# mingfeisun/DeepMimic_mujoco

Measured on AMD Instinct MI355X. Metric: env-steps/sec, higher is better.
Workload: dtype f64

## Files before the change

deepmimic_mujoco_amd/csrc/slot_kernel.h:

```cpp
#pragma once

#include <cstddef>

#include "env_kernel.h"

namespace dm {

constexpr int SLOTS = 4, SW = 16;
#ifndef DM_SLOT_MAXROWS
#define DM_SLOT_MAXROWS 40
#endif
constexpr int SLOT_MAXROWS = DM_SLOT_MAXROWS, SLOT_MAXLIMROWS = 16, SLOT_MAXCON = 13, SLOT_MAXFRAME = 8, SLOT_MAXCAND = 32, SLOT_BOXSLOTS = 3;
constexpr int SLOT_EXTROWS = SLOT_MAXROWS - 2 * SW;
static_assert(SLOT_EXTROWS == 8 || SLOT_EXTROWS == 0, "the partial third row set holds eight rows (or is absent)");
constexpr int PAIR_PASSES = MAXPAIR / SW;
static_assert(MAXPAIR <= 128 && NG <= 16, "a candidate word holds the pair number in 7 bits and both geom numbers in 4 bits each");
constexpr int DOF_PASSES = (NV + SW - 1) / SW, HINGE_PASSES = (NU + SW - 1) / SW, Q_PASSES = (NQ + SW - 1) / SW, ENT_PASSES = (310 + SW - 1) / SW;

#ifndef DM_SLOT_ASSUME
#define DM_SLOT_ASSUME 31
#endif
#ifndef DM_SLOT_A10T
#define DM_SLOT_A10T 1
#endif
// ... 594 lines not shown
        int tot_rows, tot_con;
        const int r0 = nrow + row_exclusive_scan(pc.n * rows_per, sl, lane, &tot_rows);
        const int c0 = ncon + row_exclusive_scan(pc.n, sl, lane, &tot_con);
        const unsigned fmask = dmw::row_ballot(pc.n > 0, lane);
        const int fi = nfr + __builtin_popcount(fmask & below);
        nfr += __builtin_popcount(fmask);
        if (pc.n > 0) {
          R fr[9];
          make_frame(fr, pc.nrm, pc.hint);
          if (fi < SLOT_MAXFRAME) { R* o = W.frm[fi]; for (int t = 0; t < 6; t++) o[t] = fr[t]; }
          for (int k = 0; k < pc.n; k++) {
            const int ci = c0 + k, rk = r0 + k * rows_per;
            if (ci >= SLOT_MAXCON || fi >= SLOT_MAXFRAME || rk + rows_per > MAXR) { ovf |= (ci >= SLOT_MAXCON || fi >= SLOT_MAXFRAME) ? 4 : 8; continue; }
            R cdist, cpos[3];
            if (pc.boxslot >= 0) { const R* o = W.boxc[pc.boxslot][k]; cdist = o[0]; cpos[0] = o[1]; cpos[1] = o[2]; cpos[2] = o[3]; }
            else if (k == 0) { cdist = pc.d0; cpos[0] = pc.p0[0]; cpos[1] = pc.p0[1]; cpos[2] = pc.p0[2]; }
            else { cdist = pc.d1; cpos[0] = pc.p1[0]; cpos[1] = pc.p1[1]; cpos[2] = pc.p1[2]; }
            R* o = W.con[ci];
            o[0] = cpos[0]; o[1] = cpos[1]; o[2] = cpos[2]; o[3] = cdist;
            W.coni[ci] = pidx | (fi << 8);
            for (int q = 0; q < rows_per; q++) W.rowi[rk + q] = ROW_CONTACT | (ci << 8) | (q << 16) | (dim << 20);
          }
        }
        nrow += tot_rows; ncon += tot_con;
      }
    }
  }
  if (nrow > MAXR) ovf |= 8;
  if (dmw::row_ballot(ovf != 0, lane) != 0u) { ovf |= 64; nrow = 0; ncon = 0; }
  if (sl == 0) { s.nefc = nrow; s.ncon = ncon; }
  dmw::sync();
  SLOT_RSTAMP(21)
#undef SLOT_RSTAMP
  return nrow;
}

template <int I, int NVEC, class R>
struct SlotSolveLTStep {
  static DM_DEV void run(R (*x)[NV], const R* qLD, const R* cur) {
    R nxt[14];
    dmw::reload_fence();
    load_factor_row<I - 1>(nxt, qLD);
    dmw::sched_fence();
#pragma unroll
    for (int v = 0; v < NVEC; v++) {
#pragma unroll
      for (int a = 1; a < 14; a++) { const int j = TOPO.dof_anc[I][a]; if (j >= 0) x[v][j] -= cur[a] * x[v][I]; }
      dmw::pin_value(x[v][TOPO.dof_anc[I][1]]);
    }
    SlotSolveLTStep<I - 1, NVEC, R>::run(x, qLD, nxt);
  }
};
template <int NVEC, class R> struct SlotSolveLTStep<0, NVEC, R> { static DM_DEV void run(R (*)[NV], const R*, const R*) {} };
template <int NVEC, class R> DM_DEV void slot_solve_LT(R (*x)[NV], const R* qLD) {
  R cur[14];
  dmw::reload_fence();
  load_factor_row<NV - 1>(cur, qLD);
  SlotSolveLTStep<NV - 1, NVEC, R>::run(x, qLD, cur);
}

template <int D, class R>
DM_DEV void slot_load_dof_operands(R* dst, const SlotShared<R>& s) {
  if constexpr (D < NV) {
#pragma unroll
    for (int r = 0; r < 6; r++) dst[r] = s.cdof[D][r];
    dst[6] = s.qvel[D]; dst[7] = s.qws[D];
  }
}
template <int D, int NS, class R>
struct SlotRowStep {
  static DM_DEV void run(R (*y)[NV], RowAcc<R>* ra, const SlotShared<R>& s, const R* cur) {
    R nxt[8];
    dmw::reload_fence();
    slot_load_dof_operands<D + 1>(nxt, s);
    dmw::sched_fence();
#pragma unroll
    for (int k = 0; k < NS; k++) {
      const int pb = (int)(D < 32 ? (ra[k].plus_lo >> D) & 1u : (ra[k].plus_hi >> (D - 32)) & 1u);
      const int mb = (int)(D < 32 ? (ra[k].minus_lo >> D) & 1u : (ra[k].minus_hi >> (D - 32)) & 1u);
      R j = ra[k].w[0] * cur[0] + ra[k].w[1] * cur[1] + ra[k].w[2] * cur[2] + ra[k].w[3] * cur[3] + ra[k].w[4] * cur[4] + ra[k].w[5] * cur[5];
      j = (j + ra[k].w7) * (R)(pb - mb);
      ra[k].vel += j * cur[6]; ra[k].jws += j * cur[7];
      y[k][D] = j;
      dmw::pin_value(ra[k].vel); dmw::pin_value(ra[k].jws);
    }
    SlotRowStep<D + 1, NS, R>::run(y, ra, s, nxt);
  }
};
template <int NS, class R> struct SlotRowStep<NV, NS, R> { static DM_DEV void run(R (*)[NV], RowAcc<R>*, const SlotShared<R>&, const R*) {} };

template <int CC, int NS, class R, bool T10 = false>
DM_DEV void slot_acol(R (*AR)[16 * NS], const R (*y)[NV]) {
#pragma unroll
  for (int k = 0; k < (T10 && CC < 16 ? 1 : NS); k++) {
    R acc0 = 0, acc1 = 0;
#pragma unroll
    for (int d = 0; d + 8 <= NV; d += 8) dmw::row_fmac8<CC % 16>(acc0, acc1, &y[CC / 16][d], &y[k][d]);
#pragma unroll
    for (int d = NV / 8 * 8; d < NV; d += 2) { dmw::row_fmac_old<CC % 16>(acc0, y[CC / 16][d], y[k][d]); dmw::row_fmac_old<CC % 16>(acc1, y[CC / 16][d + 1], y[k][d + 1]); }
    AR[k][CC] = acc0 + acc1;
  }
}
template <int C, int NS, class R, bool T10 = false>
struct SlotACols {
  static DM_DEV void run(R (*AR)[16 * NS], const R (*y)[NV], int nmax) {
    if constexpr (C < 16 * NS) {
      slot_acol<C, NS, R, T10>(AR, y); slot_acol<C + 1, NS, R, T10>(AR, y); slot_acol<C + 2, NS, R, T10>(AR, y); slot_acol<C + 3, NS, R, T10>(AR, y);
      if (C + 4 < nmax) SlotACols<C + 4, NS, R, T10>::run(AR, y, nmax);
    }
  }
};
// ... 186 lines not shown
  for (int r6 = 0; r6 < 6; r6++) ra.w[r6] = w[r6];
  ra.w7 = w7; ra.w8 = 0; ra.vel = 0; ra.jws = 0;
  ra.plus_lo = (unsigned)mplus; ra.plus_hi = (unsigned)(mplus >> 32); ra.minus_lo = (unsigned)mminus; ra.minus_hi = (unsigned)(mminus >> 32);
}

template <class R, int NS, bool PROF = false>
DM_DEV void slot_constraint(const DevModel<R>& M, SlotShared<R>& s, int sl_in, int lane_in, int nefc, int nmax, int& ovf, const DebugOut* dbg, long long* prof = 0) {
  const int sl = DM_SLOT_LANE_AT(4, sl_in), lane = dmw::launder(lane_in);
  long long pt0 = 0, pt1 = 0, pt_enter = 0;
  if (PROF) { pt0 = dmw::clk(); pt_enter = pt0; }
#define SLOT_STAMP(k) if constexpr (NS == 1) { DM_MARK("slot_constraint_ns1_" #k); } else if constexpr (NS == 2) { DM_MARK("slot_constraint_ns2_" #k); } else { DM_MARK("slot_constraint_ns3_" #k); } if (PROF) { pt1 = dmw::clk(); prof[k] += pt1 - pt0; pt0 = pt1; }
  constexpr bool EXT = NS == 3;
  constexpr int NF = EXT ? 2 : NS;
  constexpr int NC = 16 * NF;
  constexpr int NX = EXT ? SLOT_EXTROWS : 1;
  if constexpr (NS == 1) { DM_MARK("slot_constraint_ns1_rows"); } else if constexpr (NS == 2) { DM_MARK("slot_constraint_ns2_rows"); } else { DM_MARK("slot_constraint_ns3_rows"); }
  R y[NF + 1][NV];
  RowAcc<R> ra[NF];
  bool active[NF];
  R pos[NF], margin[NF], dA[NF], rscale[NF];
#pragma unroll
  for (int k = 0; k < NF; k++) {
    const int r = sl + 16 * k;
    active[k] = r < nefc;
    slot_row_setup(M, s, r, active[k], ra[k], pos[k], margin[k], dA[k], rscale[k]);
  }
  {
    R cur[8];
    dmw::reload_fence();
    slot_load_dof_operands<0>(cur, s);
    SlotRowStep<0, NF, R>::run(y, ra, s, cur);
  }
#pragma unroll
  for (int d = 0; d < NV; d++) y[NF][d] = s.tau[d];
  if (dbg) {
#pragma unroll
    for (int k = 0; k < NF; k++) if (active[k]) {
      double* o = dbg->out + (34 * 34 + 34 * 3 + 42 + 3) + (sl + 16 * k) * (34 + 6);
#pragma unroll
      for (int d = 0; d < NV; d++) o[d] = (double)y[k][d];
    }
  }
  SLOT_STAMP(8)
  R Rr[NF], aref[NF], f[NF];
#pragma unroll
  for (int k = 0; k < NF; k++) {
    const R imp = impedance(M, pos[k] - margin[k]);
    Rr[k] = fmax(R(DM_MINVAL), (1 - imp) * dA[k] / imp);
    if (rscale[k] != R(1)) Rr[k] = fmax(R(DM_MINVAL), rscale[k] * Rr[k]);
    aref[k] = -M.B * ra[k].vel - M.K * imp * (pos[k] - margin[k]);
    const R jar = ra[k].jws - aref[k];
    f[k] = (active[k] && jar < 0) ? -jar / Rr[k] : R(0);
  }
  slot_solve_LT<NF + 1>(y, s.r2.qLD);
#pragma unroll
  for (int d = 0; d < NV; d++) {
    const R sc = s.dsq[d];
#pragma unroll
    for (int k = 0; k <= NF; k++) { y[k][d] *= sc; dmw::pin_value(y[k][d]); }
  }
  if (dbg) {
    R x[NV];
#pragma unroll
    for (int d = 0; d < NV; d++) x[d] = y[NF][d] * s.dsq[d];
    solve_L(x, s.r2.qLD);
    if (sl == 0) {
#pragma unroll
      for (int d = 0; d < NV; d++) dbg->out[34 * 34 + 34 + d] = (double)x[d];
    }
  }
  R bb[NF];
#pragma unroll
  for (int k = 0; k < NF; k++) {
    R acc0 = 0, acc1 = 0;
#pragma unroll
    for (int d = 0; d < NV; d++) { if (d & 1) acc1 += y[k][d] * y[NF][d]; else acc0 += y[k][d] * y[NF][d]; }
    bb[k] = active[k] ? (acc0 + acc1) - aref[k] : R(0);
  }
  R y3[EXT ? NV : 1];
  bool active3 = false;
  R Rr3 = 0, f3 = 0, bb3 = 0;
  if constexpr (EXT) {
    dmw::sync();
    if (sl == 0) {
#pragma unroll
      for (int d = 0; d < NV; d++) s.tau[d] = y[NF][d];
    }
    const int r3 = 2 * SW + (sl >> 1);
    active3 = (sl & 1) == 0 && r3 < nefc;
    RowAcc<R> ra3[1];
    R pos3, margin3, dA3, rscale3;
    slot_row_setup(M, s, r3, active3, ra3[0], pos3, margin3, dA3, rscale3);
    R yy[1][NV];
    {
      R cur[8];
      dmw::reload_fence();
      slot_load_dof_operands<0>(cur, s);
      SlotRowStep<0, 1, R>::run(yy, ra3, s, cur);
    }
    const R imp = impedance(M, pos3 - margin3);
    Rr3 = fmax(R(DM_MINVAL), (1 - imp) * dA3 / imp);
    if (rscale3 != R(1)) Rr3 = fmax(R(DM_MINVAL), rscale3 * Rr3);
    const R aref3 = -M.B * ra3[0].vel - M.K * imp * (pos3 - margin3);
    const R jar = ra3[0].jws - aref3;
    f3 = (active3 && jar < 0) ? -jar / Rr3 : R(0);
    slot_solve_LT<1>(yy, s.r2.qLD);
    dmw::sync();
    R acc0 = 0, acc1 = 0;
#pragma unroll
    for (int d = 0; d < NV; d++) {
      y3[d] = yy[0][d] * s.dsq[d]; dmw::pin_value(y3[d]);
      if (d & 1) acc1 += y3[d] * s.tau[d]; else acc0 += y3[d] * s.tau[d];
    }
    bb3 = active3 ? (acc0 + acc1) - aref3 : R(0);
  }
  R U[EXT ? 2 : 1][NX], B3[NX];
  R diag3 = 1;
  if constexpr (EXT) {
#pragma unroll
    for (int j = 0; j < NX; j++) { U[0][j] = 0; U[1][j] = 0; B3[j] = 0; dmw::pin_value(U[0][j]); dmw::pin_value(U[1][j]); dmw::pin_value(B3[j]); }
    dmw::dpp_settle();
    SlotExtCols<0, R>::run(U, B3, y, y3, nmax - 2 * SW);
    R dg = 1;
#pragma unroll
    for (int j = 0; j < NX; j++) { if (sl == 2 * j) { B3[j] += active3 ? Rr3 : R(0); dg = B3[j]; } }
    diag3 = active3 ? dg : R(1);
    R* y3lds = &s.qd.o.qacc[0];
    if ((sl & 1) == 0) {
#pragma unroll
      for (int d = 0; d < NV; d++) y3lds[d * SLOT_EXTROWS + (sl >> 1)] = y3[d];
    }
  }
  SLOT_STAMP(9)
  R AR[NF][NC];
#pragma unroll
  for (int k = 0; k < NF; k++)
#pragma unroll
    for (int c = 0; c < NC; c++) { AR[k][c] = 0; dmw::pin_value(AR[k][c]); }
  dmw::dpp_settle();
  constexpr bool T10 = NS == 2 && DM_SLOT_A10T;
  SlotACols<0, NF, R, T10>::run(AR, y, nmax);
  if constexpr (T10) slot_a10_transpose(AR, s, sl);
  R diag[NF];
#pragma unroll
  for (int k = 0; k < NF; k++) {
    R dg = 1;
#pragma unroll
    for (int c = 0; c < 16; c++) { if (sl == c) { AR[k][16 * k + c] += active[k] ? Rr[k] : R(0); dg = AR[k][16 * k + c]; } }
    diag[k] = active[k] ? dg : R(1);
  }
  SLOT_STAMP(10)
  typedef decltype(dmw::park(R(0))) ParkedR;
  ParkedR ypark[NF == 2 ? NF : 1][NF == 2 ? NV : 1];
  if constexpr (NF == 2) {
    if constexpr (!EXT) {
      if (sl == 0) {
#pragma unroll
        for (int d = 0; d < NV; d++) s.tau[d] = y[NF][d];
      }
// ... 106 lines not shown
      if constexpr (EXT) nf3 = conv ? nfprev3 : nf3;
      const bool go = (int)act & (int)!conv;
      iter += go ? 1 : 0;
      anybad = (int)anybad | ((int)go & (int)bad2);
      frozen = (int)frozen | (int)conv;
      chg = chg2;
      more = dmw::ballot(!frozen) != 0ull;
      if (PROF) prof[6] += 1;
    }
  }
#pragma unroll
  for (int k = 0; k < NF; k++) f[k] = -nf[k];
  f3 = -nf3;
  if (PROF && NS >= 2) { prof[22] += dmw::clk() - pt0; }
  if (PROF && NS == 3) { prof[27] += dmw::clk() - pt0; }
  SLOT_STAMP(12)
  if (PROF) { prof[14] += nmax; prof[15] += 1; }
  if (dmw::row_ballot(anybad, lane) != 0u) ovf |= 16 | 64;
  if (dbg) {
#pragma unroll
    for (int k = 0; k < NF; k++) if (active[k]) {
      double* o = dbg->out + (34 * 34 + 34 * 3 + 42 + 3) + (sl + 16 * k) * (34 + 6) + 34;
      o[0] = (double)pos[k]; o[1] = (double)margin[k]; o[2] = (double)Rr[k]; o[3] = (double)aref[k]; o[4] = (double)bb[k]; o[5] = (double)f[k];
    }
  }
  R fy3[EXT ? NV : 1];
  if constexpr (EXT) {
    const R* y3lds = &s.qd.o.qacc[0];
    const R f3a = active3 ? f3 : R(0);
#pragma unroll
    for (int d = 0; d < NV; d++) { fy3[d] = ((sl & 1) == 0 ? y3lds[d * SLOT_EXTROWS + (sl >> 1)] : R(0)) * f3a; dmw::pin_value(fy3[d]); }
  }
  if constexpr (NF == 2) {
    dmw::sync();
#pragma unroll
    for (int d = 0; d < NV; d++) y[NF][d] = s.tau[d];
  }
#pragma unroll
  for (int k = 0; k < NF; k++) {
    const R fk = active[k] ? f[k] : R(0);
#pragma unroll
    for (int d = 0; d < NV; d++) { if constexpr (NF == 2) y[k][d] = dmw::unpark(ypark[k][d]); y[k][d] *= fk; dmw::pin_value(y[k][d]); }
  }
  R ws[NV];
#pragma unroll
  for (int d = 0; d < NV; d++) { ws[d] = 0; dmw::pin_value(ws[d]); }
  R one = 1;
  dmw::pin_value(one);
  dmw::dpp_settle();
  SlotAssemble<0, NF, R>::run(ws, y, one, nmax);
  if constexpr (EXT) SlotExtAssemble<0, R>::run(ws, fy3, one, nmax - 2 * SW);
#pragma unroll
  for (int d = 0; d < NV; d++) ws[d] = (ws[d] + y[NF][d]) * s.dsq[d];
  solve_L(ws, s.r2.qLD);
  if (sl == 0) {
#pragma unroll
    for (int d = 0; d < NV; d++) s.qd.o.qacc[d] = ws[d];
    s.solver_iter = iter;
  }
  dmw::sync();
  SLOT_STAMP(13)
  if (PROF && NS >= 2) prof[24] += dmw::clk() - pt_enter;
  if (PROF && NS == 3) prof[26] += dmw::clk() - pt_enter;
#undef SLOT_STAMP
}

#if !defined(DM_WAVE_TESTBENCH)
template <class R, int MAXR>
static __device__ __noinline__ int slot_rows_call(const DevModel<R>* M, SlotShared<R>* s, int sl, int lane, int* ovf) {
  int o = *ovf;
  const int n = slot_rows<R, false, MAXR>(*dmw::in_constant(M), *dmw::in_lds(s), sl, lane, o, (long long*)0);
  *ovf = o;
  return n;
}
#endif

template <class R>
DM_DEV void slot_smooth_solve(SlotShared<R>& s, int sl, const DebugOut* dbg) {
  R x[1][NV];
#pragma unroll
  for (int d = 0; d < NV; d++) x[0][d] = s.tau[d];
  slot_solve_LT<1>(x, s.r2.qLD);
#pragma unroll
  for (int d = 0; d < NV; d++) { x[0][d] *= s.dsq[d]; dmw::pin_value(x[0][d]); }
#pragma unroll
  for (int d = 0; d < NV; d++) x[0][d] = (R(0) + x[0][d]) * s.dsq[d];
  solve_L(x[0], s.r2.qLD);
  if (sl == 0) {
#pragma unroll
    for (int d = 0; d < NV; d++) { s.qd.o.qacc[d] = x[0][d]; if (dbg) dbg->out[34 * 34 + 34 + d] = (double)x[0][d]; }
    s.solver_iter = 0;
  }
  dmw::sync();
}

template <class R, bool PROF = false, bool CARRY = false, int MAXR = 2 * SW>
DM_DEV void slot_forward(const DevModel<R>& M, SlotShared<R>& s, const SlotTables& tb, int sl, int lane, const LaneTopo& lt, R* xip, int& ovf, const DebugOut* dbg, long long* prof = 0) {
  long long t0 = 0, t1 = 0;
  if (PROF) t0 = dmw::clk();
#define SLOT_FSTAMP(k) if (PROF) { t1 = dmw::clk(); prof[k] += t1 - t0; t0 = t1; }
  DM_MARK("slot_kinematics");
  bool skip_kin = false;
  if constexpr (CARRY) {
    skip_kin = dmw::ballot(s.kin_ok() != R(0)) == ~0ull;
    dmw::sync();
    if (sl == 0) s.kin_ok() = R(0);
  }
  if (!skip_kin) slot_kinematics(M, s, sl, lt, xip);
  SLOT_FSTAMP(0)
  if (dbg) { for (int e = sl; e < NV * NV; e += SW) dbg->out[e] = 0; dmw::sync(); }
  DM_MARK("slot_bias");
  slot_bias(M, s, tb, sl, lt);
  SLOT_FSTAMP(1)
  if (dbg) {
    for (int c = 0; c < DOF_PASSES; c++) { const int d = sl + SW * c; if (d < NV) dbg->out[34 * 34 + d] = (double)(-M.dof_damping[d] * s.qvel[d] + s.act[d] - s.tau[d]); }
  }
  DM_MARK("slot_mass_factor");
  slot_mass_matrix<R, PROF>(M, s, tb, sl, lt, dbg, prof);
  SLOT_FSTAMP(2)
  DM_MARK("slot_rows");
  int nefc = 0;
#if !defined(DM_WAVE_TESTBENCH)
  if (!PROF && (M.enable_contact || M.enable_limit)) nefc = slot_rows_call<R, MAXR>(&M, &s, sl, lane, &ovf);
  else
#endif
  if (M.enable_contact || M.enable_limit) nefc = slot_rows<R, PROF, MAXR>(M, s, sl, lane, ovf, prof);
  else { if (sl == 0) { s.nefc = 0; s.ncon = 0; } dmw::sync(); }
  SLOT_FSTAMP(3)
  DM_MARK("slot_constraint");
  const int nmax = rows_max(nefc);
  if (nmax == 0) slot_smooth_solve(s, sl, dbg);
#ifdef DM_FORCE_EXT
  else if (nmax > 0 && MAXR > 2 * SW) slot_constraint<R, MAXR > 2 * SW ? 3 : 2, PROF>(M, s, sl, lane, nefc, nmax > 2 * SW ? nmax : 2 * SW + 1, ovf, dbg, prof);
#endif
  else if (nmax <= 16) slot_constraint<R, 1, PROF>(M, s, sl, lane, nefc, nmax, ovf, dbg, prof);
  else if (nmax <= 2 * SW) { slot_constraint<R, 2, PROF>(M, s, sl, lane, nefc, nmax, ovf, dbg, prof); if (PROF) prof[7] += 1; }
  else if constexpr (MAXR > 2 * SW) { slot_constraint<R, 3, PROF>(M, s, sl, lane, nefc, nmax, ovf, dbg, prof); if (PROF) { prof[7] += 1; prof[25] += 1; } }
  SLOT_FSTAMP(4)
  DM_MARK("slot_forward_end");
#undef SLOT_FSTAMP
// ... 9 lines not shown
```

deepmimic_mujoco_amd/csrc/slot_step.h:

```cpp
#pragma once

#include "env_step.h"
#include "slot_kernel.h"

namespace dm {

template <class R> struct DofVec { R r[DOF_PASSES]; };

template <class R>
DM_DEV void slot_integrate_pos(SlotShared<R>& s, const DofVec<R>& x0q, int sl, R h) {
  const R q0 = dmw::row_bcast<3>(x0q.r[0]), q1 = dmw::row_bcast<4>(x0q.r[0]), q2 = dmw::row_bcast<5>(x0q.r[0]), q3 = dmw::row_bcast<6>(x0q.r[0]);
  if (sl < 3) s.qpos[sl] = x0q.r[0] + h * s.tau[sl];
  else if (sl == 3) {
    R ax[3] = {s.tau[3], s.tau[4], s.tau[5]}, q[4] = {q0, q1, q2, q3}, qr[4];
    const R angle = h * normalize3(ax);
    if (angle == R(0)) { qr[0] = 1; qr[1] = qr[2] = qr[3] = 0; } else axisangle2quat(qr, ax, angle);
    normalize4(q);
    quat_mul(q, q, qr);
    s.qpos[3] = q[0]; s.qpos[4] = q[1]; s.qpos[5] = q[2]; s.qpos[6] = q[3];
  } else if (sl >= 7) s.qpos[sl] = x0q.r[0] + h * s.tau[sl - 1];
#pragma unroll
  for (int c = 1; c < Q_PASSES; c++) { const int i = sl + SW * c; if (i < NQ) s.qpos[i] = x0q.r[c] + h * s.tau[i - 1]; }
}

// ... 55 lines not shown
    if (i < NQ) s.qpos[i] = B.qpos[(size_t)env * NQ + i];
    if (i < NV) { s.qvel[i] = B.qvel[(size_t)env * NV + i]; s.qws[i] = B.qws[(size_t)env * NV + i]; s.act[i] = 0; }
  }
  if (sl == 0) { s.status = 0; s.nefc = 0; s.ncon = 0; s.solver_iter = 0; }
  dmw::sync();
  if (action) {
#pragma unroll
    for (int c = 0; c < HINGE_PASSES; c++) {
      const int u = sl + SW * c;
      if (u < NU) {
        const R a = ctrl_of_action(M, B, env, u, (R)action[(size_t)env * NU + u], s.qpos[7 + u], s.qvel[6 + u], n_substeps);
        if (live) B.ctrl[(size_t)env * NU + u] = a;
        s.act[u + 6] = act_force(M, u + 6, a);
      }
    }
  }
  dmw::sync_mem();
}

template <class R, bool CARRY = false>
DM_DEV void slot_spd_control(const DevModel<R>& M, const Batch<R>& B, SlotShared<R>& s, const SlotTables& tb, int env, int sl, const LaneTopo& lt, bool live,
                             const DofVec<R>& qbar, const DofVec<R>& vbar) {
  const R h = M.timestep;
#pragma unroll
  for (int c = 0; c < DOF_PASSES; c++) { const int d = sl + SW * c; if (d < NV) s.act[d] = 0; }
  dmw::sync();
  R xip[3];
  bool skip_kin = false;
  if constexpr (CARRY) {
    skip_kin = dmw::ballot(s.kin_ok() != R(0)) == ~0ull;
    dmw::sync();
    if (sl == 0) s.kin_ok() = R(0);
  }
  if (!skip_kin) slot_kinematics(M, s, sl, lt, xip);
  slot_bias(M, s, tb, sl, lt);
  slot_mass_matrix<R, false, true>(M, s, tb, sl, lt, (const DebugOut*)0);
  R pd[DOF_PASSES], kd[DOF_PASSES];
#pragma unroll
  for (int c = 0; c < DOF_PASSES; c++) {
    const int d = sl + SW * c;
    pd[c] = 0; kd[c] = 0;
    if (d >= 6 && d < NV) {
      const R q = s.qpos[d + 1], v = s.qvel[d];
      kd[c] = M.kd[d];
      pd[c] = M.kp[d] * (qbar.r[c] - q - h * v) + kd[c] * (vbar.r[c] - v);
      s.tau[d] += pd[c];
    }
  }
  dmw::sync();
  {
    R x[1][NV];
#pragma unroll
    for (int d = 0; d < NV; d++) x[0][d] = s.tau[d];
    slot_solve_LT<1>(x, s.r2.qLD);
#pragma unroll
    for (int d = 0; d < NV; d++) { x[0][d] *= s.qd.o.dinv[d]; dmw::pin_value(x[0][d]); }
    solve_L(x[0], s.r2.qLD);
    if (sl == 0) {
#pragma unroll
      for (int d = 0; d < NV; d++) s.qd.o.qacc[d] = x[0][d];
    }
  }
  dmw::sync();
#pragma unroll
  for (int c = 0; c < DOF_PASSES; c++) {
    const int d = sl + SW * c;
    if (d >= 6 && d < NV) {
      const R ct = spd_ctrl(M, d, pd[c], kd[c], s.qd.o.qacc[d], h);
      if (live) B.ctrl[(size_t)env * NU + (d - 6)] = ct;
      s.act[d] = act_force(M, d, ct);
    }
  }
  dmw::sync_mem();
}

template <class R>
DM_DEV void slot_store_state(const Batch<R>& B, SlotShared<R>& s, int env, int sl, bool live) {
  if (!live) return;
#pragma unroll
  for (int c = 0; c < Q_PASSES; c++) {
    const int i = sl + SW * c;
    if (i < NQ) B.qpos[(size_t)env * NQ + i] = s.qpos[i];
    if (i < NV) { B.qvel[(size_t)env * NV + i] = s.qvel[i]; B.qws[(size_t)env * NV + i] = s.qws[i]; }
  }
}

template <class R>
DM_DEV void slot_reset_env(const DevModel<R>& M, const Batch<R>& B, SlotShared<R>& s, int env, int sl, bool doit, int mode, int hard) {
  const int ep = B.episode[env];
  const int genv = B.env_offset + env;
  const int idx = reset_draw(B, env, ep);
  if (doit) {
#pragma unroll
    for (int c = 0; c < Q_PASSES; c++) {
      const int i = sl + SW * c;
      if (i < NQ) {
        R q, v = 0;
        reset_element(M, B, mode, idx, genv, ep, i, q, v);
        s.qpos[i] = q;
        if (i < NV) s.qvel[i] = v;
      }
      if (hard && i < NV) s.qws[i] = 0;
    }
  }
  dmw::sync_mem();
  if (doit && sl == 0) reset_commit(B, env, ep, mode, hard, idx);
}
template <class R>
DM_DEV void slot_reset_env_clips(const DevModel<R>& M, const Batch<R>& B, const ClipArgs<R>& C, SlotShared<R>& s, int env, int sl, bool doit, int mode, int hard) {
  const int c = C.episode_clip(B, env, B.episode[env], mode, hard);
// ... 320 lines not shown
```

deepmimic_mujoco_amd/csrc/wave.h:

```cpp
#pragma once

#if defined(DM_WAVE_TESTBENCH)
#include "wave_testbench.h"
#else
#include <hip/hip_runtime.h>

#define DM_DEV __device__ __forceinline__
#define DM_DEV_NOINLINE __device__ __noinline__
#ifndef DM_NO_STATIC_CALLS
#define DM_STATIC_CALLS 1
#define DM_DEV_CALL64 static __device__ __noinline__
#else
#define DM_DEV_CALL64 __device__ __noinline__
#endif
#define DM_CONSTANT __device__ constexpr

namespace dmw {
DM_DEV int lane() { return (int)(threadIdx.x & 63u); }
DM_DEV void sync() { __builtin_amdgcn_fence(__ATOMIC_SEQ_CST, "wavefront"); __builtin_amdgcn_wave_barrier(); }
DM_DEV void sync_mem() { __syncthreads(); }
DM_DEV unsigned long long ballot(bool p) { return __ballot(p); }
DM_DEV int shfl_i(int v, int src) { return __shfl(v, src, 64); }
DM_DEV double shfl(double v, int src) { return __shfl(v, src, 64); }
DM_DEV float shfl(float v, int src) { return __shfl(v, src, 64); }
// ... 67 lines not shown
}
template <class T> DM_DEV T* in_lds(T* p) {
#if defined(__HIP_DEVICE_COMPILE__)
  __builtin_assume(__builtin_amdgcn_is_shared((const void*)p));
#endif
  return p;
}
template <class T> DM_DEV T* in_global(T* p) {
  __attribute__((address_space(1))) T* g = (__attribute__((address_space(1))) T*)uniform_ptr(p);
  asm volatile("" : "+s"(g));
  return (T*)g;
}
template <class T> DM_DEV const T* in_constant(const T* p) {
  __attribute__((address_space(4))) const T* g = (__attribute__((address_space(4))) const T*)uniform_ptr(p);
  asm volatile("" : "+s"(g));
  return (const T*)g;
}
template <class T> DM_DEV T* launder_uniform_ptr(T* p) { asm volatile("" : "+s"(p)); return p; }
DM_DEV void reload_fence() { asm volatile("" ::: "memory"); }
DM_DEV void lds_sub(bool pred, double* p, double v) { if (pred) __hip_atomic_fetch_add(p, -v, __ATOMIC_RELAXED, __HIP_MEMORY_SCOPE_WORKGROUP); }
DM_DEV void lds_sub(bool pred, float* p, float v) { if (pred) __hip_atomic_fetch_add(p, -v, __ATOMIC_RELAXED, __HIP_MEMORY_SCOPE_WORKGROUP); }
template <int I> DM_DEV double row_bcast(double v) {
  long long x = __double_as_longlong(v);
  x = __builtin_amdgcn_update_dpp(0ll, x, 0x150 + I, 0xf, 0xf, true);
  return __longlong_as_double(x);
}
template <int I> DM_DEV float row_bcast(float v) { return __int_as_float(__builtin_amdgcn_update_dpp(0, __float_as_int(v), 0x150 + I, 0xf, 0xf, true)); }
template <int I> DM_DEV int row_bcast_i(int v) { return __builtin_amdgcn_update_dpp(0, v, 0x150 + I, 0xf, 0xf, true); }
template <int I> DM_DEV void row_fmac(double& acc, double x, double y) {
  asm volatile("s_nop 1\n\tv_fmac_f64_dpp %0, %1, %2 row_newbcast:%3 row_mask:0xf bank_mask:0xf" : "+v"(acc) : "v"(x), "v"(y), "n"(I));
}
template <int I> DM_DEV void row_fmac(float& acc, float x, float y) { acc += row_bcast<I>(x) * y; }
template <int I> DM_DEV void row_fmac_old(double& acc, double x, double y) {
  asm volatile("s_nop 1\n\tv_fmac_f64_dpp %0, %1, %2 row_newbcast:%3 row_mask:0xf bank_mask:0xf" : "+v"(acc) : "v"(x), "v"(y), "n"(I));
}
template <int I> DM_DEV void row_fmac_old(float& acc, float x, float y) { acc += row_bcast<I>(x) * y; }
#define DM_FMAC_DPP(acc, x, y) "v_fmac_f64_dpp " acc ", " x ", " y " row_newbcast:%18 row_mask:0xf bank_mask:0xf\n\t"
template <int I> DM_DEV void row_fmac8(double& acc0, double& acc1, const double* x, const double* y) {
  asm volatile("s_nop 1\n\t" DM_FMAC_DPP("%0", "%2", "%10") DM_FMAC_DPP("%1", "%3", "%11") DM_FMAC_DPP("%0", "%4", "%12") DM_FMAC_DPP("%1", "%5", "%13")
               DM_FMAC_DPP("%0", "%6", "%14") DM_FMAC_DPP("%1", "%7", "%15") DM_FMAC_DPP("%0", "%8", "%16") DM_FMAC_DPP("%1", "%9", "%17")
               : "+v"(acc0), "+v"(acc1)
               : "v"(x[0]), "v"(x[1]), "v"(x[2]), "v"(x[3]), "v"(x[4]), "v"(x[5]), "v"(x[6]), "v"(x[7]),
                 "v"(y[0]), "v"(y[1]), "v"(y[2]), "v"(y[3]), "v"(y[4]), "v"(y[5]), "v"(y[6]), "v"(y[7]), "n"(I));
}
#undef DM_FMAC_DPP
#define DM_FMAC_DPP(acc, x) "v_fmac_f64_dpp " acc ", " x ", %16 row_newbcast:%17 row_mask:0xf bank_mask:0xf\n\t"
template <int I> DM_DEV void row_add8(double* a, const double* x, double one) {
  asm volatile("s_nop 1\n\t" DM_FMAC_DPP("%0", "%8") DM_FMAC_DPP("%1", "%9") DM_FMAC_DPP("%2", "%10") DM_FMAC_DPP("%3", "%11")
               DM_FMAC_DPP("%4", "%12") DM_FMAC_DPP("%5", "%13") DM_FMAC_DPP("%6", "%14") DM_FMAC_DPP("%7", "%15")
               : "+v"(a[0]), "+v"(a[1]), "+v"(a[2]), "+v"(a[3]), "+v"(a[4]), "+v"(a[5]), "+v"(a[6]), "+v"(a[7])
               : "v"(x[0]), "v"(x[1]), "v"(x[2]), "v"(x[3]), "v"(x[4]), "v"(x[5]), "v"(x[6]), "v"(x[7]), "v"(one), "n"(I));
}
#undef DM_FMAC_DPP
template <int I> DM_DEV void row_fmac8(float& acc0, float& acc1, const float* x, const float* y) { for (int k = 0; k < 8; k++) { if (k & 1) acc1 += row_bcast<I>(x[k]) * y[k]; else acc0 += row_bcast<I>(x[k]) * y[k]; } }
template <int I> DM_DEV void row_add8(float* a, const float* x, float one) { for (int k = 0; k < 8; k++) a[k] += row_bcast<I>(x[k]) * one; }
template <int I> DM_DEV void pgs_row(double& t, double& tsave, double nf0, double a, double onehot) {
  double delta;
  asm volatile("v_max_f64 %0, %3, %1\n\tv_fma_f64 %2, %5, %1, %2\n\ts_nop 0\n\tv_fmac_f64_dpp %1, %0, %4 row_newbcast:%6 row_mask:0xf bank_mask:0xf"
               : "=&v"(delta), "+v"(t), "+v"(tsave) : "v"(nf0), "v"(a), "v"(onehot), "n"(I));
}
template <int I> DM_DEV void pgs_row2(double& t_own, double& tsave_own, double& t_other, double nf0, double a_own, double a_other, double onehot) {
  double delta;
  asm volatile("v_max_f64 %0, %4, %1\n\tv_fma_f64 %2, %7, %1, %2\n\ts_nop 0\n\tv_fmac_f64_dpp %1, %0, %5 row_newbcast:%8 row_mask:0xf bank_mask:0xf\n\t"
               "v_fmac_f64_dpp %3, %0, %6 row_newbcast:%8 row_mask:0xf bank_mask:0xf"
               : "=&v"(delta), "+v"(t_own), "+v"(tsave_own), "+v"(t_other) : "v"(nf0), "v"(a_own), "v"(a_other), "v"(onehot), "n"(I));
}
template <int I> DM_DEV void pgs_row3(double& t3, double& tsave3, double& t0, double& t1, double nf0, double b, double u0, double u1, double onehot) {
  double delta;
  asm volatile("v_max_f64 %0, %5, %1\n\tv_fma_f64 %2, %9, %1, %2\n\ts_nop 0\n\tv_fmac_f64_dpp %1, %0, %6 row_newbcast:%10 row_mask:0xf bank_mask:0xf\n\t"
               "v_fmac_f64_dpp %3, %0, %7 row_newbcast:%10 row_mask:0xf bank_mask:0xf\n\tv_fmac_f64_dpp %4, %0, %8 row_newbcast:%10 row_mask:0xf bank_mask:0xf"
               : "=&v"(delta), "+v"(t3), "+v"(tsave3), "+v"(t0), "+v"(t1) : "v"(nf0), "v"(b), "v"(u0), "v"(u1), "v"(onehot), "n"(I));
}
template <int I> DM_DEV void pgs_row3(float& t3, float& tsave3, float& t0, float& t1, float nf0, float b, float u0, float u1, float onehot) {
  const float d = max_raw(nf0, t3); tsave3 += onehot * t3; const float bc = row_bcast<I>(d); t3 += bc * b; t0 += bc * u0; t1 += bc * u1;
}
#define DM_PGS1(D, A, OH, I) "v_max_f64 " D ", %3, %0\n\tv_fma_f64 %1, " OH ", %0, %1\n\ts_nop 0\n\tv_fmac_f64_dpp %0, " D ", " A " row_newbcast:" I " row_mask:0xf bank_mask:0xf\n\t"
template <int I0> DM_DEV void pgs_rows4(double& t, double& tsave, double nf0, const double* a, const double* oh) {
  double d;
  asm volatile(DM_PGS1("%2", "%4", "%8", "%12") DM_PGS1("%2", "%5", "%9", "%13") DM_PGS1("%2", "%6", "%10", "%14") DM_PGS1("%2", "%7", "%11", "%15")
               : "+v"(t), "+v"(tsave), "=&v"(d)
               : "v"(nf0), "v"(a[0]), "v"(a[1]), "v"(a[2]), "v"(a[3]), "v"(oh[0]), "v"(oh[1]), "v"(oh[2]), "v"(oh[3]), "n"(I0), "n"(I0 + 1), "n"(I0 + 2), "n"(I0 + 3));
}
#undef DM_PGS1
template <int I0> DM_DEV void pgs_rows4_2(double& t_own, double& tsave_own, double& t_other, double nf0, const double* a_own, const double* a_other, const double* oh) {
  double d0, d1;
  asm volatile(
      "v_max_f64 %3, %5, %0\n\tv_fma_f64 %1, %14, %0, %1\n\ts_nop 0\n\tv_fmac_f64_dpp %0, %3, %6 row_newbcast:%18 row_mask:0xf bank_mask:0xf\n\t"
      "v_max_f64 %4, %5, %0\n\tv_fma_f64 %1, %15, %0, %1\n\tv_fmac_f64_dpp %2, %3, %10 row_newbcast:%18 row_mask:0xf bank_mask:0xf\n\tv_fmac_f64_dpp %0, %4, %7 row_newbcast:%19 row_mask:0xf bank_mask:0xf\n\t"
      "v_max_f64 %3, %5, %0\n\tv_fma_f64 %1, %16, %0, %1\n\tv_fmac_f64_dpp %2, %4, %11 row_newbcast:%19 row_mask:0xf bank_mask:0xf\n\tv_fmac_f64_dpp %0, %3, %8 row_newbcast:%20 row_mask:0xf bank_mask:0xf\n\t"
      "v_max_f64 %4, %5, %0\n\tv_fma_f64 %1, %17, %0, %1\n\tv_fmac_f64_dpp %2, %3, %12 row_newbcast:%20 row_mask:0xf bank_mask:0xf\n\tv_fmac_f64_dpp %0, %4, %9 row_newbcast:%21 row_mask:0xf bank_mask:0xf\n\t"
      "s_nop 0\n\tv_fmac_f64_dpp %2, %4, %13 row_newbcast:%21 row_mask:0xf bank_mask:0xf"
      : "+v"(t_own), "+v"(tsave_own), "+v"(t_other), "=&v"(d0), "=&v"(d1)
      : "v"(nf0), "v"(a_own[0]), "v"(a_own[1]), "v"(a_own[2]), "v"(a_own[3]), "v"(a_other[0]), "v"(a_other[1]), "v"(a_other[2]), "v"(a_other[3]),
        "v"(oh[0]), "v"(oh[1]), "v"(oh[2]), "v"(oh[3]), "n"(I0), "n"(I0 + 1), "n"(I0 + 2), "n"(I0 + 3));
}
template <int I> DM_DEV void pgs_row(float& t, float& tsave, float nf0, float a, float onehot) { const float d = max_raw(nf0, t); tsave += onehot * t; t += row_bcast<I>(d) * a; }
template <int I> DM_DEV void pgs_row2(float& t_own, float& tsave_own, float& t_other, float nf0, float a_own, float a_other, float onehot) {
  const float d = max_raw(nf0, t_own); tsave_own += onehot * t_own; const float b = row_bcast<I>(d); t_own += b * a_own; t_other += b * a_other;
}
template <int I0> DM_DEV void pgs_rows4(float& t, float& tsave, float nf0, const float* a, const float* oh) {
  pgs_row<I0>(t, tsave, nf0, a[0], oh[0]); pgs_row<I0 + 1>(t, tsave, nf0, a[1], oh[1]); pgs_row<I0 + 2>(t, tsave, nf0, a[2], oh[2]); pgs_row<I0 + 3>(t, tsave, nf0, a[3], oh[3]);
}
template <int I0> DM_DEV void pgs_rows4_2(float& t_own, float& tsave_own, float& t_other, float nf0, const float* a_own, const float* a_other, const float* oh) {
  pgs_row2<I0>(t_own, tsave_own, t_other, nf0, a_own[0], a_other[0], oh[0]); pgs_row2<I0 + 1>(t_own, tsave_own, t_other, nf0, a_own[1], a_other[1], oh[1]);
  pgs_row2<I0 + 2>(t_own, tsave_own, t_other, nf0, a_own[2], a_other[2], oh[2]); pgs_row2<I0 + 3>(t_own, tsave_own, t_other, nf0, a_own[3], a_other[3], oh[3]);
}
DM_DEV void dpp_settle() { asm volatile("s_nop 4"); }
struct Parked { int lo, hi; };
DM_DEV Parked park(double v) {
  Parked p;
  asm volatile("v_accvgpr_write_b32 %0, %2\n\tv_accvgpr_write_b32 %1, %3" : "=a"(p.lo), "=a"(p.hi) : "v"(__double2loint(v)), "v"(__double2hiint(v)));
  return p;
}
DM_DEV double unpark(const Parked& p) {
  int lo, hi;
  asm volatile("v_accvgpr_read_b32 %0, %2\n\tv_accvgpr_read_b32 %1, %3" : "=v"(lo), "=v"(hi) : "a"(p.lo), "a"(p.hi));
  return __hiloint2double(hi, lo);
}
struct ParkedF { int x; };
DM_DEV ParkedF park(float v) { ParkedF p; asm volatile("v_accvgpr_write_b32 %0, %1" : "=a"(p.x) : "v"(__float_as_int(v))); return p; }
DM_DEV float unpark(const ParkedF& p) { int x; asm volatile("v_accvgpr_read_b32 %0, %1" : "=v"(x) : "a"(p.x)); return __int_as_float(x); }
DM_DEV int global_counter_next(int* p) { return atomicAdd(p, 1); }
DM_DEV unsigned row_ballot(bool p, int lane_id) { return (unsigned)((__ballot(p) >> (lane_id & 48)) & 0xffffull); }
}
#endif

namespace dmw {
DM_DEV double sum8(double v) { v += perm_xor1(v); v += perm_xor2(v); v += perm_half_mirror(v); return v; }
DM_DEV double sum16(double v) { v = sum8(v); v += perm_row_mirror(v); return v; }
DM_DEV double wave_sum(double v) {
  v = sum16(v);
  return ((bcast(v, 0) + bcast(v, 16)) + bcast(v, 32)) + bcast(v, 48);
}
#if !defined(DM_WAVE_TESTBENCH)
DM_DEV float sum8(float v) { v += perm_xor1(v); v += perm_xor2(v); v += perm_half_mirror(v); return v; }
DM_DEV float sum16(float v) { v = sum8(v); v += perm_row_mirror(v); return v; }
DM_DEV float wave_sum(float v) {
  v = sum16(v);
  return ((bcast(v, 0) + bcast(v, 16)) + bcast(v, 32)) + bcast(v, 48);
}
#endif
DM_DEV int wave_exclusive_scan(int v, int lane_id, int* total) {
  const unsigned long long below = (1ull << lane_id) - 1ull;
  int pre = 0, tot = 0;
#pragma unroll
  for (int b = 0; b < 5; b++) {
    const unsigned long long m = ballot(((v >> b) & 1) != 0);
    pre += __builtin_popcountll(m & below) << b;
    tot += __builtin_popcountll(m) << b;
  }
  *total = tot;
  return pre;
}
}
```

Before: 21.22 million.

## Spread factor rows across lanes and broadcast via DPP in slot triangular solves

The slot L^T and L triangular solves used to load each factor row's ancestor entries into per-lane registers (14 loads per row) from LDS. Now each lane loads a single lane-offset word of the row, with a prefetch queue of configurable depth. The entries are applied through DPP row_newbcast fmac instructions in inline asm, which cuts per-row LDS loads and register pressure. The cost is hand-written asm chains, clamped lane addressing that relies on a static bound check, and a dependence on the DPP broadcast semantics.

```diff
diff --git a/deepmimic_mujoco_amd/csrc/slot_kernel.h b/deepmimic_mujoco_amd/csrc/slot_kernel.h
--- a/deepmimic_mujoco_amd/csrc/slot_kernel.h
+++ b/deepmimic_mujoco_amd/csrc/slot_kernel.h
@@ -670,11 +670,82 @@
   }
 };
 template <int NVEC, class R> struct SlotSolveLTStep<0, NVEC, R> { static DM_DEV void run(R (*)[NV], const R*, const R*) {} };
-template <int NVEC, class R> DM_DEV void slot_solve_LT(R (*x)[NV], const R* qLD) {
-  R cur[14];
-  dmw::reload_fence();
-  load_factor_row<NV - 1>(cur, qLD);
-  SlotSolveLTStep<NV - 1, NVEC, R>::run(x, qLD, cur);
+#ifndef DM_SLOT_LT_BCAST
+#define DM_SLOT_LT_BCAST 1
+#endif
+#ifndef DM_SLOT_LT_AHEAD
+#define DM_SLOT_LT_AHEAD 2
+#endif
+constexpr int SLOT_LT_AHEAD = DM_SLOT_LT_AHEAD;
+constexpr int SLOT_LT_LANE_CLAMP = 14;
+constexpr int max_dof_depth() { int m = 0; for (int i = 0; i < NV; i++) if (TOPO.dof_depth[i] > m) m = TOPO.dof_depth[i]; return m; }
+static_assert(max_dof_depth() - 1 <= 13 && SLOT_LT_LANE_CLAMP >= max_dof_depth() - 1 && SLOT_LT_LANE_CLAMP < SW && elim_unmasked_reads_fit(),
+              "every ancestor number a row names is a lane at or below the clamp, and the clamped lane-indexed read of every row stays inside qLD[312]");
+template <int I> struct DofAnc { static constexpr int at(int a) { return TOPO.dof_anc[I][a]; } };
+template <int I, class R> DM_DEV R slot_factor_word(const R* qLD_lane) { if constexpr (I >= 1 && I < NV) return qLD_lane[TOPO.madr[I]]; else return R(0); }
+template <int I, int NVEC, class R>
+struct SlotSolveLTBcastStep {
+  static DM_DEV void run(R (*x)[NV], const R* qLD_lane, R* pre) {
+    dmw::reload_fence();
+    const R cur = pre[0];
+#pragma unroll
+    for (int k = 0; k + 1 < SLOT_LT_AHEAD; k++) pre[k] = pre[k + 1];
+    pre[SLOT_LT_AHEAD - 1] = slot_factor_word<I - SLOT_LT_AHEAD>(qLD_lane);
+    dmw::sched_fence();
+#pragma unroll
+    for (int v = 0; v < NVEC; v++) {
+      dmw::row_fnmac_lanes<TOPO.dof_depth[I] - 1, DofAnc<I>>(x[v], cur, x[v][I]);
+      dmw::pin_value(x[v][TOPO.dof_anc[I][1]]);
+    }
+    SlotSolveLTBcastStep<I - 1, NVEC, R>::run(x, qLD_lane, pre);
+  }
+};
+template <int NVEC, class R> struct SlotSolveLTBcastStep<0, NVEC, R> { static DM_DEV void run(R (*)[NV], const R*, R*) {} };
+template <int NVEC, class R> DM_DEV void slot_solve_LT(R (*x)[NV], const R* qLD, int sl) {
+  if constexpr (DM_SLOT_LT_BCAST) {
+    const R* qLD_lane = qLD + (sl < SLOT_LT_LANE_CLAMP ? sl : SLOT_LT_LANE_CLAMP);
+    R pre[SLOT_LT_AHEAD];
+    dmw::reload_fence();
+#pragma unroll
+    for (int k = 0; k < SLOT_LT_AHEAD; k++) pre[k] = qLD_lane[TOPO.madr[NV - 1 - k]];
+    SlotSolveLTBcastStep<NV - 1, NVEC, R>::run(x, qLD_lane, pre);
+  } else {
+    R cur[14];
+    dmw::reload_fence();
+    load_factor_row<NV - 1>(cur, qLD);
+    SlotSolveLTStep<NV - 1, NVEC, R>::run(x, qLD, cur);
+  }
+}
+
+#ifndef DM_SLOT_L_BCAST
+#define DM_SLOT_L_BCAST 1
+#endif
+template <int I, class R>
+struct SlotSolveLBcastStep {
+  static DM_DEV void run(R* x, const R* qLD_lane, R* pre) {
+    dmw::reload_fence();
+    const R cur = pre[0];
+#pragma unroll
+    for (int k = 0; k + 1 < SLOT_LT_AHEAD; k++) pre[k] = pre[k + 1];
+    pre[SLOT_LT_AHEAD - 1] = slot_factor_word<I + SLOT_LT_AHEAD>(qLD_lane);
+    dmw::sched_fence();
+    R acc0 = 0, acc1 = 0;
+    dmw::row_fmac_lanes<TOPO.dof_depth[I] - 1, DofAnc<I>>(acc0, acc1, x, cur);
+    x[I] -= acc0 + acc1;
+    dmw::pin_value(x[I]);
+    SlotSolveLBcastStep<I + 1, R>::run(x, qLD_lane, pre);
+  }
+};
+template <class R> struct SlotSolveLBcastStep<NV, R> { static DM_DEV void run(R*, const R*, R*) {} };
+template <class R> DM_DEV void slot_solve_L(R* x, const R* qLD, int sl) {
+  if constexpr (DM_SLOT_L_BCAST) {
+    const R* qLD_lane = qLD + (sl < SLOT_LT_LANE_CLAMP ? sl : SLOT_LT_LANE_CLAMP);
+    R pre[SLOT_LT_AHEAD];
+    dmw::reload_fence();
+#pragma unroll
+    for (int k = 0; k < SLOT_LT_AHEAD; k++) pre[k] = qLD_lane[TOPO.madr[1 + k]];
+    SlotSolveLBcastStep<1, R>::run(x, qLD_lane, pre);
+  } else solve_L(x, qLD);
 }
 
 template <int D, class R>
@@ -967,7 +1038,7 @@
     const R jar = ra[k].jws - aref[k];
     f[k] = (active[k] && jar < 0) ? -jar / Rr[k] : R(0);
   }
-  slot_solve_LT<NF + 1>(y, s.r2.qLD);
+  slot_solve_LT<NF + 1>(y, s.r2.qLD, sl);
 #pragma unroll
   for (int d = 0; d < NV; d++) {
     const R sc = s.dsq[d];
@@ -978,7 +1049,7 @@
     R x[NV];
 #pragma unroll
     for (int d = 0; d < NV; d++) x[d] = y[NF][d] * s.dsq[d];
-    solve_L(x, s.r2.qLD);
+    slot_solve_L(x, s.r2.qLD, sl);
     if (sl == 0) {
 #pragma unroll
       for (int d = 0; d < NV; d++) dbg->out[34 * 34 + 34 + d] = (double)x[d];
@@ -1019,7 +1090,7 @@
     const R aref3 = -M.B * ra3[0].vel - M.K * imp * (pos3 - margin3);
     const R jar = ra3[0].jws - aref3;
     f3 = (active3 && jar < 0) ? -jar / Rr3 : R(0);
-    slot_solve_LT<1>(yy, s.r2.qLD);
+    slot_solve_LT<1>(yy, s.r2.qLD, sl);
     dmw::sync();
     R acc0 = 0, acc1 = 0;
 #pragma unroll
@@ -1232,7 +1303,7 @@
   if constexpr (EXT) SlotExtAssemble<0, R>::run(ws, fy3, one, nmax - 2 * SW);
 #pragma unroll
   for (int d = 0; d < NV; d++) ws[d] = (ws[d] + y[NF][d]) * s.dsq[d];
-  solve_L(ws, s.r2.qLD);
+  slot_solve_L(ws, s.r2.qLD, sl);
   if (sl == 0) {
 #pragma unroll
     for (int d = 0; d < NV; d++) s.qd.o.qacc[d] = ws[d];
@@ -1260,12 +1331,12 @@
   R x[1][NV];
 #pragma unroll
   for (int d = 0; d < NV; d++) x[0][d] = s.tau[d];
-  slot_solve_LT<1>(x, s.r2.qLD);
+  slot_solve_LT<1>(x, s.r2.qLD, sl);
 #pragma unroll
   for (int d = 0; d < NV; d++) { x[0][d] *= s.dsq[d]; dmw::pin_value(x[0][d]); }
 #pragma unroll
   for (int d = 0; d < NV; d++) x[0][d] = (R(0) + x[0][d]) * s.dsq[d];
-  solve_L(x[0], s.r2.qLD);
+  slot_solve_L(x[0], s.r2.qLD, sl);
   if (sl == 0) {
 #pragma unroll
     for (int d = 0; d < NV; d++) { s.qd.o.qacc[d] = x[0][d]; if (dbg) dbg->out[34 * 34 + 34 + d] = (double)x[0][d]; }
diff --git a/deepmimic_mujoco_amd/csrc/slot_step.h b/deepmimic_mujoco_amd/csrc/slot_step.h
--- a/deepmimic_mujoco_amd/csrc/slot_step.h
+++ b/deepmimic_mujoco_amd/csrc/slot_step.h
@@ -131,10 +131,10 @@
     R x[1][NV];
 #pragma unroll
     for (int d = 0; d < NV; d++) x[0][d] = s.tau[d];
-    slot_solve_LT<1>(x, s.r2.qLD);
+    slot_solve_LT<1>(x, s.r2.qLD, sl);
 #pragma unroll
     for (int d = 0; d < NV; d++) { x[0][d] *= s.qd.o.dinv[d]; dmw::pin_value(x[0][d]); }
-    solve_L(x[0], s.r2.qLD);
+    slot_solve_L(x[0], s.r2.qLD, sl);
     if (sl == 0) {
 #pragma unroll
       for (int d = 0; d < NV; d++) s.qd.o.qacc[d] = x[0][d];
diff --git a/deepmimic_mujoco_amd/csrc/wave.h b/deepmimic_mujoco_amd/csrc/wave.h
--- a/deepmimic_mujoco_amd/csrc/wave.h
+++ b/deepmimic_mujoco_amd/csrc/wave.h
@@ -143,6 +143,130 @@
                : "v"(x[0]), "v"(x[1]), "v"(x[2]), "v"(x[3]), "v"(x[4]), "v"(x[5]), "v"(x[6]), "v"(x[7]), "v"(one), "n"(I));
 }
 #undef DM_FMAC_DPP
+#define DM_NF(k, a) "v_fmac_f64_dpp %" #k ", %[L], -%[X] row_newbcast:" #a " row_mask:0xf bank_mask:0xf\n\t"
+#define DM_NF1 DM_NF(0, 1)
+#define DM_NF2 DM_NF1 DM_NF(1, 2)
+#define DM_NF3 DM_NF2 DM_NF(2, 3)
+#define DM_NF4 DM_NF3 DM_NF(3, 4)
+#define DM_NF5 DM_NF4 DM_NF(4, 5)
+#define DM_NF6 DM_NF5 DM_NF(5, 6)
+#define DM_NF7 DM_NF6 DM_NF(6, 7)
+#define DM_NF8 DM_NF7 DM_NF(7, 8)
+#define DM_NF9 DM_NF8 DM_NF(8, 9)
+#define DM_NF10 DM_NF9 DM_NF(9, 10)
+#define DM_NF11 DM_NF10 DM_NF(10, 11)
+#define DM_NF12 DM_NF11 DM_NF(11, 12)
+#define DM_NF13 DM_NF12 DM_NF(12, 13)
+#define DM_NA(a) "+v"(x[ANC::at(a)])
+#define DM_NA1 DM_NA(1)
+#define DM_NA2 DM_NA1, DM_NA(2)
+#define DM_NA3 DM_NA2, DM_NA(3)
+#define DM_NA4 DM_NA3, DM_NA(4)
+#define DM_NA5 DM_NA4, DM_NA(5)
+#define DM_NA6 DM_NA5, DM_NA(6)
+#define DM_NA7 DM_NA6, DM_NA(7)
+#define DM_NA8 DM_NA7, DM_NA(8)
+#define DM_NA9 DM_NA8, DM_NA(9)
+#define DM_NA10 DM_NA9, DM_NA(10)
+#define DM_NA11 DM_NA10, DM_NA(11)
+#define DM_NA12 DM_NA11, DM_NA(12)
+#define DM_NA13 DM_NA12, DM_NA(13)
+#define DM_NCASE(n) if constexpr (N == n) asm volatile("s_nop 1\n\t" DM_NF##n : DM_NA##n : [L] "v"(L), [X] "v"(xi));
+template <int N, class ANC> DM_DEV void row_fnmac_lanes(double* x, double L, double xi) {
+  static_assert(N >= 0 && N <= 13, "a factor row has at most thirteen ancestors");
+  DM_NCASE(1) DM_NCASE(2) DM_NCASE(3) DM_NCASE(4) DM_NCASE(5) DM_NCASE(6) DM_NCASE(7) DM_NCASE(8) DM_NCASE(9) DM_NCASE(10) DM_NCASE(11) DM_NCASE(12) DM_NCASE(13)
+}
+#undef DM_NCASE
+#undef DM_NA
+#undef DM_NF
+#undef DM_NF1
+#undef DM_NA1
+#undef DM_NF2
+#undef DM_NA2
+#undef DM_NF3
+#undef DM_NA3
+#undef DM_NF4
+#undef DM_NA4
+#undef DM_NF5
+#undef DM_NA5
+#undef DM_NF6
+#undef DM_NA6
+#undef DM_NF7
+#undef DM_NA7
+#undef DM_NF8
+#undef DM_NA8
+#undef DM_NF9
+#undef DM_NA9
+#undef DM_NF10
+#undef DM_NA10
+#undef DM_NF11
+#undef DM_NA11
+#undef DM_NF12
+#undef DM_NA12
+#undef DM_NF13
+#undef DM_NA13
+#define DM_PF(acc, k, a) "v_fmac_f64_dpp " acc ", %[L], %" #k " row_newbcast:" #a " row_mask:0xf bank_mask:0xf\n\t"
+#define DM_PF1 DM_PF("%0", 2, 1)
+#define DM_PF2 DM_PF1 DM_PF("%1", 3, 2)
+#define DM_PF3 DM_PF2 DM_PF("%0", 4, 3)
+#define DM_PF4 DM_PF3 DM_PF("%1", 5, 4)
+#define DM_PF5 DM_PF4 DM_PF("%0", 6, 5)
+#define DM_PF6 DM_PF5 DM_PF("%1", 7, 6)
+#define DM_PF7 DM_PF6 DM_PF("%0", 8, 7)
+#define DM_PF8 DM_PF7 DM_PF("%1", 9, 8)
+#define DM_PF9 DM_PF8 DM_PF("%0", 10, 9)
+#define DM_PF10 DM_PF9 DM_PF("%1", 11, 10)
+#define DM_PF11 DM_PF10 DM_PF("%0", 12, 11)
+#define DM_PF12 DM_PF11 DM_PF("%1", 13, 12)
+#define DM_PF13 DM_PF12 DM_PF("%0", 14, 13)
+#define DM_PX(a) "v"(x[ANC::at(a)])
+#define DM_PX1 DM_PX(1)
+#define DM_PX2 DM_PX1, DM_PX(2)
+#define DM_PX3 DM_PX2, DM_PX(3)
+#define DM_PX4 DM_PX3, DM_PX(4)
+#define DM_PX5 DM_PX4, DM_PX(5)
+#define DM_PX6 DM_PX5, DM_PX(6)
+#define DM_PX7 DM_PX6, DM_PX(7)
+#define DM_PX8 DM_PX7, DM_PX(8)
+#define DM_PX9 DM_PX8, DM_PX(9)
+#define DM_PX10 DM_PX9, DM_PX(10)
+#define DM_PX11 DM_PX10, DM_PX(11)
+#define DM_PX12 DM_PX11, DM_PX(12)
+#define DM_PX13 DM_PX12, DM_PX(13)
+#define DM_PCASE(n) if constexpr (N == n) asm volatile("s_nop 1\n\t" DM_PF##n : "+v"(acc0), "+v"(acc1) : DM_PX##n, [L] "v"(L));
+template <int N, class ANC> DM_DEV void row_fmac_lanes(double& acc0, double& acc1, const double* x, double L) {
+  static_assert(N >= 1 && N <= 13, "a factor row has at most thirteen ancestors");
+  DM_PCASE(1) DM_PCASE(2) DM_PCASE(3) DM_PCASE(4) DM_PCASE(5) DM_PCASE(6) DM_PCASE(7) DM_PCASE(8) DM_PCASE(9) DM_PCASE(10) DM_PCASE(11) DM_PCASE(12) DM_PCASE(13)
+}
+#undef DM_PCASE
+#undef DM_PX
+#undef DM_PF
+#undef DM_PF1
+#undef DM_PX1
+#undef DM_PF2
+#undef DM_PX2
+#undef DM_PF3
+#undef DM_PX3
+#undef DM_PF4
+#undef DM_PX4
+#undef DM_PF5
+#undef DM_PX5
+#undef DM_PF6
+#undef DM_PX6
+#undef DM_PF7
+#undef DM_PX7
+#undef DM_PF8
+#undef DM_PX8
+#undef DM_PF9
+#undef DM_PX9
+#undef DM_PF10
+#undef DM_PX10
+#undef DM_PF11
+#undef DM_PX11
+#undef DM_PF12
+#undef DM_PX12
+#undef DM_PF13
+#undef DM_PX13
 template <int I> DM_DEV void row_fmac8(float& acc0, float& acc1, const float* x, const float* y) { for (int k = 0; k < 8; k++) { if (k & 1) acc1 += row_bcast<I>(x[k]) * y[k]; else acc0 += row_bcast<I>(x[k]) * y[k]; } }
 template <int I> DM_DEV void row_add8(float* a, const float* x, float one) { for (int k = 0; k < 8; k++) a[k] += row_bcast<I>(x[k]) * one; }
 template <int I> DM_DEV void pgs_row(double& t, double& tsave, double nf0, double a, double onehot) {
@@ -217,6 +341,22 @@
 #endif
 
 namespace dmw {
+template <int A, int N, class ANC, class T> DM_DEV void row_fnmac_lanes_from(T* x, T L, T nxi) {
+  if constexpr (A <= N) { x[ANC::at(A)] = x[ANC::at(A)] + row_bcast<A>(L) * nxi; row_fnmac_lanes_from<A + 1, N, ANC, T>(x, L, nxi); }
+}
+template <int A, int N, class ANC, class T> DM_DEV void row_fmac_lanes_from(T& acc0, T& acc1, const T* x, T L) {
+  if constexpr (A <= N) {
+    if constexpr (A & 1) acc0 = acc0 + row_bcast<A>(L) * x[ANC::at(A)]; else acc1 = acc1 + row_bcast<A>(L) * x[ANC::at(A)];
+    row_fmac_lanes_from<A + 1, N, ANC, T>(acc0, acc1, x, L);
+  }
+}
+#if defined(DM_WAVE_TESTBENCH)
+template <int N, class ANC, class T> DM_DEV void row_fnmac_lanes(T* x, T L, T xi) { row_fnmac_lanes_from<1, N, ANC, T>(x, L, -xi); }
+template <int N, class ANC, class T> DM_DEV void row_fmac_lanes(T& acc0, T& acc1, const T* x, T L) { row_fmac_lanes_from<1, N, ANC, T>(acc0, acc1, x, L); }
+#else
+template <int N, class ANC> DM_DEV void row_fnmac_lanes(float* x, float L, float xi) { row_fnmac_lanes_from<1, N, ANC, float>(x, L, -xi); }
+template <int N, class ANC> DM_DEV void row_fmac_lanes(float& acc0, float& acc1, const float* x, float L) { row_fmac_lanes_from<1, N, ANC, float>(acc0, acc1, x, L); }
+#endif
 DM_DEV double sum8(double v) { v += perm_xor1(v); v += perm_xor2(v); v += perm_half_mirror(v); return v; }
 DM_DEV double sum16(double v) { v = sum8(v); v += perm_row_mirror(v); return v; }
 DM_DEV double wave_sum(double v) {
```

After: 21.00 million. 1.0% lower.
